# thenumbernine/lua-multigrid-poisson

Measured on AMD Instinct MI355X. Metric: V-cycles/sec + finest-smoother achieved HBM GB/s, 3D Poisson, higher is better.
Workload: dtype f32; 1 GPU; BASELINE configs[2]: 3D Poisson 512^3 per GPU, 7-point, RB-GS 2+2, V-cycle, trilinear P, 2x2x2-average R, consistent coarse boundary, per-cycle RMS-update err; parallelism=single GPU, levels=10

## Files before the change

lua-multigrid-poisson_amd/csrc/mgp_internal.h:

```cpp
#pragma once
#include <hip/hip_runtime.h>
#include <cstdint>

namespace mgp {

constexpr int kGhost3D = 1;
constexpr int kGhostZs = 5;
constexpr int kZsHaloPre = 5, kZsHaloPost = 4, kZsHaloCoarse = 3;

struct Geo {
    int nx, ny;
    int lx, ly;
    int hw, lhw;
    int64_t nz;
    int64_t H;
    int64_t P;
    int64_t z0;
    int64_t gnz;
};

constexpr int kRealF32D = 12;

hipError_t launch_init_point_charge(int rb, int dim, void* u, void* f, Geo g, int64_t cx, int64_t cy,
                                    int64_t cz, hipStream_t s);
// ... 11 lines not shown
                             const void* old, double* partials, Geo g, double h, double cl, bool gs, hipStream_t s);
bool fresh_supported(int rb, const Geo& g);
hipError_t launch_fresh_sweep(int rb, int dim, const void* f, void* u, Geo g, double h, double cl, hipStream_t s,
                              bool store_red = true);
bool post1_supported(int rb, const Geo& g, const Geo& gc);
hipError_t launch_post_first(int rb, int dim, int linear, void* u, const void* V, const void* f, Geo g, Geo gc,
                             double h, double cl, double clc, hipStream_t s);
hipError_t launch_residual_restrict(int rb, int dim, const void* u, const void* f, void* R, Geo g, Geo gc, double h,
                                    double cl, hipStream_t s);
bool bres_supported(int rb, const Geo& g);
hipError_t launch_black_residual_restrict(int rb, int dim, void* u, const void* f, void* R, Geo g, Geo gc, double h,
                                          double cl, hipStream_t s);
hipError_t launch_rb_sweep(int rb, int dim, const void* src, const void* f, void* dst, Geo g, double h, double cl,
                           bool store_red, hipStream_t s);
hipError_t launch_residual_field_v(int rb, int dim, const void* u, const void* f, void* r, Geo g, double h, double cl,
                                   hipStream_t s);
hipError_t launch_fw_restrict(int rb, int dim, const void* r, void* R, Geo g, Geo gc, double clc, hipStream_t s);
bool resfw_supported(int rb, int dim, const Geo& g, int gz, bool dist);
hipError_t launch_resfw(int rb, int dim, const void* u, const void* f, void* R, Geo g, Geo gc, double h, double cl,
                        double clc, int gz, hipStream_t s);
hipError_t launch_prolong_correct(int rb, int dim, int linear, void* u, const void* V, Geo g, Geo gc, double clc,
                                  hipStream_t s, bool black_only = false);
hipError_t launch_sqdiff_sum(int rb, const void* a, const void* b, int64_t n, double* partials, double* out,
                             hipStream_t s, int* ctr = nullptr);
hipError_t launch_nonfinite_check(int rb, const void* p, int64_t n, int id, int* first, hipStream_t s);
hipError_t launch_metrics(int rb, const void* psi, const void* old, int64_t n, double* partials, double* out,
                          hipStream_t s);
int resnorm_blocks(int rb, Geo g);
hipError_t launch_residual_norm(int rb, int dim, const void* u, const void* f, Geo g, double h, double cl,
                                double* partials, double* out, hipStream_t s);
int sum_scratch(int n);
hipError_t launch_sum_partials(const double* partials, int n, double* out, hipStream_t s, int* ctr = nullptr);

int defect_blocks(Geo g);
int refine_add_blocks(Geo g);
int refine_partials();
hipError_t launch_defect(int dim, const double* psi64, const double* f64, float* r32, float* u32_or_null, Geo g,
                         double h, double* partials, double* out, hipStream_t s);
hipError_t launch_refine_add(double* psi64, const float* e32, Geo g, double* partials, double* out, hipStream_t s);
hipError_t launch_refine_widen(const float* src, double* dst, int64_t n, hipStream_t s);
hipError_t launch_refine_narrow(const double* src, float* dst, int64_t n, hipStream_t s);

struct FusedTuning {
    bool wide = true;
    int ys_half = -1;
    int ys_rows = 32;
    int64_t wgs = 256;
    int patch_pre = 0, patch_post = -1;
    bool fwf = true;
    int post_zc = 256;
    bool split = true;
    bool split_cl = false;
    bool zpost_pre = true;
    bool stamp_r = false;
};
FusedTuning fused_tuning_from_env();

struct LaunchInfo {
    char name[96];
    int64_t grid;
};

struct FusedArgs {
    FusedTuning tu;
    LaunchInfo* info;
    bool pre;
    int linear;
    const void* src;
    const void* f;
    void* dst;
    const void* old;
    void* R;
    const void* V;
    double* partials;
    Geo g, gc;
    double h, cl, clc;
    int zc;
    int ghost;
};
bool fused_supported(int rb, int dim, int ns, const Geo& g, const FusedTuning& tu);
hipError_t prepare_kernels(int rb);
int fused_zc(int rb, const Geo& g, bool pre, bool clz, const FusedTuning& tu);
int fused_blocks(int rb, const Geo& g, int zc, bool clz, const FusedTuning& tu);
hipError_t launch_fused(int rb, const FusedArgs& a, hipStream_t s);
bool fused_fwf_supported(int rb, int dim, bool clz, bool dist, const FusedTuning& tu);

constexpr int kBlkMaxSweeps = 2;
constexpr int kBlkTile = 8;
constexpr int kBlkTile2D = 32;
struct BlockArgs {
    bool pre;
    int linear;
    int ns;
    const void* src;
    const void* f;
    void* dst;
    void* R;
    const void* V;
    Geo g, gc;
    double h, cl, clc;
};
bool block_supported(int rb, int dim, int ns, const Geo& g);
hipError_t launch_block(int rb, int dim, const BlockArgs& a, hipStream_t s);

struct Block2Args {
    bool pre;
// ... 62 lines not shown
```

lua-multigrid-poisson_amd/csrc/mgp_kernels.hip:

```cpp
#include "mgp_device.h"

#include <cstdio>
#include <cstdlib>
#include <type_traits>
#include <utility>

namespace mgp {
namespace {




constexpr unsigned kMaxBlocks = 1u << 20;
inline unsigned nblk_gs(int64_t n)
{
    const int64_t b = (n + kBlock - 1) / kBlock;
    return (unsigned)(b < (int64_t)kMaxBlocks ? (b > 0 ? b : 1) : kMaxBlocks);
}

template <typename T>
__global__ __launch_bounds__(kBlock) void k_init(T* __restrict__ u, T* __restrict__ f, Geo g, int64_t cx, int64_t cy,
                                                 int64_t cz, int dim3)
{
    const int64_t n = g.P * g.nz;
// ... 1232 lines not shown
#endif
#ifndef ZS_TYPRE_CL_F32
#define ZS_TYPRE_CL_F32 ZS_TYPRE_F32
#endif
#ifndef ZS_NPRE_CL_F32
#define ZS_NPRE_CL_F32 ZS_NPRE_F32
#endif
#ifndef ZS_TXPOST_W_F32
#define ZS_TXPOST_W_F32 128
#endif
#ifndef ZS_TYPOST_W_F32
#define ZS_TYPOST_W_F32 16
#endif
#ifndef ZS_NPOST_W_F32
#define ZS_NPOST_W_F32 ZS_NPOST_F32
#endif
template <typename T>
struct ZsTile;
template <>
struct ZsTile<float> {
    static constexpr int TXPRE = ZS_TXPRE_F32, TXPOST = ZS_TXPOST_F32, TYPRE = ZS_TYPRE_F32, TYPOST = ZS_TYPOST_F32,
                         NPRE = ZS_NPRE_F32, NPOST = ZS_NPOST_F32;
    static constexpr int TXPRE_CL = ZS_TXPRE_CL_F32, TYPRE_CL = ZS_TYPRE_CL_F32, NPRE_CL = ZS_NPRE_CL_F32;
    static constexpr int TXPOST_W = ZS_TXPOST_W_F32, TYPOST_W = ZS_TYPOST_W_F32, NPOST_W = ZS_NPOST_W_F32;
};
#ifndef ZS_TXPRE_F64
#define ZS_TXPRE_F64 32
#endif
#ifndef ZS_TXPOST_F64
#define ZS_TXPOST_F64 64
#endif
#ifndef ZS_TYPRE_F64
#define ZS_TYPRE_F64 32
#endif
#ifndef ZS_TYPOST_F64
#define ZS_TYPOST_F64 16
#endif
template <>
struct ZsTile<double> {
    static constexpr int TXPRE = ZS_TXPRE_F64, TXPOST = ZS_TXPOST_F64, TYPRE = ZS_TYPRE_F64, TYPOST = ZS_TYPOST_F64,
                         NPRE = 2, NPOST = 2;
    static constexpr int TXPRE_CL = TXPRE, TYPRE_CL = TYPRE, NPRE_CL = NPRE;
    static constexpr int TXPOST_W = TXPOST, TYPOST_W = TYPOST, NPOST_W = NPOST;
};
#ifndef ZS_NT
#define ZS_NT 0
#endif
constexpr bool kZsNTL = (ZS_NT & 1) != 0, kZsNTS = (ZS_NT & 2) != 0, kZsNTO = (ZS_NT & 5) != 0;
#ifndef ZS_PRE_RED_STORE
#define ZS_PRE_RED_STORE 0
#endif
constexpr bool kZsPreRed = ZS_PRE_RED_STORE != 0;

template <typename T, bool PRE, bool CLZ = true, bool WIDE = false, bool FWF = false>
struct ZsShape {
    static constexpr int N = PRE ? (CLZ ? ZsTile<T>::NPRE : ZsTile<T>::NPRE_CL)
                                 : (WIDE ? ZsTile<T>::NPOST_W : ZsTile<T>::NPOST);
    static constexpr int TX = PRE ? (CLZ ? ZsTile<T>::TXPRE : ZsTile<T>::TXPRE_CL)
                                  : (WIDE ? ZsTile<T>::TXPOST_W : ZsTile<T>::TXPOST);
    static constexpr int TY = PRE ? (CLZ ? ZsTile<T>::TYPRE : ZsTile<T>::TYPRE_CL)
                                  : (WIDE ? ZsTile<T>::TYPOST_W : ZsTile<T>::TYPOST);
    static constexpr int H = PRE ? (FWF ? 6 : 5) : 4;
#ifdef ZS_HX_FIXED
    static constexpr int HX = ZS_HX_FIXED;
#else
    static constexpr int HX = 2 * N * ((H + 2 * N - 1) / (2 * N));
#endif
    static constexpr int HWE = (TX + 2 * HX) / 2;
    static constexpr int G = HWE / N;
    static constexpr int HXG = HX / 2 / N;
    static constexpr int YE = TY + 2 * H;
    static constexpr int NT = G * YE;
    static constexpr int YEV = (YE + 1) / 2;
    static constexpr int NPAR = (G * YEV + 63) / 64 * 64;
    static constexpr bool PS = PRE ? ZS_PSPLIT_PRE != 0 : ZS_PSPLIT_POST != 0;
    static constexpr int NTL = PS ? 2 * NPAR : (NT + 63) / 64 * 64;
    static constexpr int YT0 = TY * G, YT1 = YT0 + 6 * G, YT2S = (YT1 + 63) / 64 * 64, YT2 = YT2S + 4 * G;
    static constexpr bool YROLE = ZS_YROLE && PRE && !PS && H == 5 && (YT2 + 63) / 64 * 64 <= NTL;
    static constexpr int GC = G - 2 * HXG, TC = TY * GC;
    static constexpr bool XROLE = YROLE && ZS_XROLE && TC % 64 == 0;
    static constexpr bool XPAIR = XROLE && ZS_XPAIR && GC == 8 && TY % 8 == 0 && HWE == 40;
    static __device__ __forceinline__ int xp_row(int q) { return (0x54450110 >> (4 * q)) & 15; }
    static __device__ __forceinline__ int xp_gx(int q) { return (0x64024620 >> (4 * q)) & 15; }
    static __device__ __forceinline__ int yrow(int t)
    {
        if (!YROLE) return t < NT ? t / G : -1;
        if (XPAIR && t < TC) return H + 8 * (t >> 6) + xp_row((t & 31) >> 2) + 2 * ((t >> 5) & 1);
        if (t < YT0) return H + (XROLE ? (t < TC ? t / GC : (t - TC) / (2 * HXG)) : t / G);
        if (t < YT1) {
            const int r = (t - YT0) / G;
            return r < 3 ? H - 3 + r : H + TY + r - 3;
        }
        if (t >= YT2S && t < YT2) {
            const int r = (t - YT2S) / G;
            return r < 2 ? H - 5 + r : H + TY + r + 1;
        }
        return -1;
    }
    static __device__ __forceinline__ int ycol(int t)
    {
        if (XROLE && t < YT0) {
            if (t < TC) return HXG + (XPAIR ? ((xp_gx((t & 31) >> 2) + (t & 3)) & 7) : t % GC);
            const int k = (t - TC) % (2 * HXG);
            return k < HXG ? k : GC + k;
        }
        return YROLE && t >= YT2S ? (t - YT2S) % G : t % G;
    }
    static constexpr int wave_role(int w)
    {
        return !YROLE || 64 * w < (XROLE ? TC : YT0) ? 0 : (64 * w < YT1 ? 1 : 2);
// ... 1169 lines not shown
#pragma unroll
            for (int e = 0; e < N; ++e) {
                rr[0][e] = pq == 0 ? rred[e] : rblk[e];
                rr[1][e] = pq == 0 ? rblk[e] : rred[e];
            }
            const int dq = q - (ST ? (Z0 & ~1) : Z0);
            if (dq >= 0 && dq <= zc && tile_xy)
                zs_restrict_avg<T, N>(rr, xr, acc, dq, zc, even_row, xs(q), R, (zz0 + q - 1) >> 1, gy >> 1, col.gm, cz0, gc);
            FB[sl(5)] = fb;
        }
    };

    if (wk == 0) {
        const int wrole = S::wave_role(lw);
        run(prefetch_a, [&](auto st, auto rt, const PF& cur, PF& nxt, int p) __attribute__((always_inline)) {
            step_a(st, rt, cur, nxt, p, decltype(st)::value ? wrole : 0);
        });
    } else if (wk == 1) {
        if (lw < SP::NTW)
            run(prefetch_b, [&](auto st, auto rt, const PF& cur, PF& nxt, int p) __attribute__((always_inline)) {
                step_b(st, rt, STY, p);
            });
        else
            run(prefetch_b, [&](auto st, auto rt, const PF& cur, PF& nxt, int p) __attribute__((always_inline)) {
                step_b(st, rt, GEN, p);
            });
    } else {
        run(
            [&](auto st, PF& r, int p) __attribute__((always_inline)) {
                if (!grp_b) prefetch_a(st, r, p);
            },
            [&](auto st, auto rt, const PF& cur, PF& nxt, int p) __attribute__((always_inline)) {
                if (!grp_b) step_a(st, rt, cur, nxt, p, 2);
                asm volatile("" ::: "memory");
                if (grp_b) step_b(st, rt, GEN, p);
            });
    }
}

template <typename T, bool ZSRC>
__global__ __launch_bounds__((ZsSplit<T>::NTL)) void k_zs_split(const T* __restrict__ src, const T* __restrict__ f,
                                                                 T* __restrict__ dst, T* __restrict__ R, Geo g, Geo gc,
                                                                 Op<T, 3> op, int zc, int gz, int patch)
{
    zs_split_body<T, ZSRC, true>(src, f, dst, R, g, gc, op, zc, gz, patch);
}

template <typename T>
__global__ __launch_bounds__((ZsSplit<T>::NTL)) void k_zs_split_cl(const T* __restrict__ f, T* __restrict__ dst,
                                                                    T* __restrict__ R, Geo g, Geo gc, Op<T, 3> op, int zc,
                                                                    int gz, int patch)
{
    zs_split_body<T, true, false>(nullptr, f, dst, R, g, gc, op, zc, gz, patch);
}

#ifndef YS_TX_F32
#define YS_TX_F32 1024
#endif
#ifndef YS_TX_F64
#define YS_TX_F64 512
#endif
template <typename T>
constexpr int ys_tx_full() { return sizeof(T) == 4 ? YS_TX_F32 : YS_TX_F64; }
template <typename T, bool PRE, int TXV = ys_tx_full<T>()>
struct YsShape {
    static constexpr int N = 16 / sizeof(T);
    static constexpr int TX = TXV;
    static constexpr int H = PRE ? 5 : 4;
    static constexpr int HX = 2 * N * ((H + 2 * N - 1) / (2 * N));
    static constexpr int HWE = TX / 2 + HX;
    static constexpr int G = HWE / N;
    static constexpr int HXG = HX / 2 / N;
    static constexpr int NTL = (G + 63) / 64 * 64;
    static constexpr int ES = 2 * G;
    static constexpr int OFF1 = 2 * ES, OFF2 = 4 * ES, OFF3 = 6 * ES, OFF4 = 10 * ES;
    static constexpr int CI = PRE ? 0 : TX / 2 + 16, CPAIRS = CI / 2, OFFC = 12 * ES;
    static constexpr size_t lds_floats = 12 * ES + 4 * CI;
    static_assert(CPAIRS <= 2 * NTL, "coarse staging: two pairs per thread");
    static_assert(NTL <= 1024, "too many threads");
    static_assert(2 * N * HXG >= H, "x halo too small");
};

#ifndef YS_PF
#define YS_PF 2
#endif
static_assert(YS_PF >= 1 && YS_PF <= 3, "prefetch distance 1..3");
template <typename T>
struct YsPrefetch {
    static constexpr int N = 16 / sizeof(T);
    Vec<T, N> u, f1, f2, o0, o1;
    Vec<T, 2> cv[2];
};

template <typename T, int N, bool CLZ, bool RES, bool AIN = false>
__device__ __forceinline__ void ys_cells(const Vec<T, N>& ym, const Vec<T, N>& cen, const Vec<T, N>& yp, T ep, T en,
                                         const Vec<T, N>& fv, const Vec<T, N>& uc, int o, int nby, int gm, int nx,
                                         bool xin, const Op<T, 2>& op, T (&out)[N], T (&ask)[N])
{
    if (!AIN) {
        ZsNb<T, N> nb;
        nb.yl = ym;
        nb.yr = yp;
        nb.ep = ep;
        nb.en = en;
        T t[N];
        zs_xsum<T, N>(cen, nb, o, t);
// ... 1673 lines not shown
template <int D>
static hipError_t pr_f32d(int linear, void* u, const void* V, Geo g, Geo gc, double clc, bool black, hipStream_t s)
{
    for (int color = black ? 1 : 0; color < 2; ++color) {
        const unsigned nb = nblk(g.H * g.nz);
        if (linear) k_prolong<float, D, 1, double><<<nb, kBlock, 0, s>>>((float*)u, (const float*)V, g, gc, clc, color);
        else k_prolong<float, D, 0, double><<<nb, kBlock, 0, s>>>((float*)u, (const float*)V, g, gc, clc, color);
        const hipError_t e = hipGetLastError();
        if (e != hipSuccess) return e;
    }
    return hipSuccess;
}

hipError_t launch_prolong_correct(int rb, int dim, int linear, void* u, const void* V, Geo g, Geo gc, double clc,
                                  hipStream_t s, bool black_only)
{
    if (rb == kRealF32D)
        return dim == 3 ? pr_f32d<3>(linear, u, V, g, gc, clc, black_only, s) : pr_f32d<2>(linear, u, V, g, gc, clc, black_only, s);
    if (rb == 8)
        return dim == 3 ? pr_t<double, 3>(linear, u, V, g, gc, clc, black_only, s)
                        : pr_t<double, 2>(linear, u, V, g, gc, clc, black_only, s);
    return dim == 3 ? pr_t<float, 3>(linear, u, V, g, gc, clc, black_only, s)
                    : pr_t<float, 2>(linear, u, V, g, gc, clc, black_only, s);
}


static int parse_patch(const char* v, int dflt)
{
    int px = 0, py = 0;
    if (!v) return dflt;
    if (std::sscanf(v, "%d,%d", &px, &py) != 2 || px < 1 || py < 1 || px > 255 || py > 255) return 0;
    return px | (py << 8);
}

FusedTuning fused_tuning_from_env()
{
    FusedTuning t;
    if (const char* v = std::getenv("MGP_ZS_WIDE")) t.wide = std::atoi(v) != 0;
    if (const char* v = std::getenv("MGP_YS_HALF")) t.ys_half = std::atoi(v);
    if (const char* v = std::getenv("MGP_YS_ROWS")) {
        const int r = std::atoi(v);
        t.ys_rows = r >= 8 && (r & 1) == 0 ? r : 32;
    }
    if (const char* v = std::getenv("MGP_ZS_WGS")) t.wgs = std::max<int64_t>(1, std::atoll(v));
    const char* vb = std::getenv("MGP_ZS_PATCH");
    const int both = parse_patch(vb, 0);
    t.patch_pre = parse_patch(std::getenv("MGP_ZS_PATCH_PRE"), both);
    t.patch_post = parse_patch(std::getenv("MGP_ZS_PATCH_POST"), vb ? both : -1);
    if (const char* v = std::getenv("MGP_ZS_FWF")) t.fwf = std::atoi(v) != 0;
    if (const char* v = std::getenv("MGP_ZS_POST_ZC")) t.post_zc = std::max(0, std::atoi(v));
    if (const char* v = std::getenv("MGP_ZS_SPLIT")) t.split = std::atoi(v) != 0;
    if (const char* v = std::getenv("MGP_ZS_SPLIT_CL")) t.split_cl = std::atoi(v) != 0;
    if (const char* v = std::getenv("MGP_ZPOST_PRE")) t.zpost_pre = std::atoi(v) != 0;
    if (const char* v = std::getenv("MGP_STAMP_R")) t.stamp_r = std::atoi(v) != 0;
    return t;
}

static int zs_patch(int patch, int tiles_x, int tiles_y, unsigned nb)
{
    if (patch == -1) patch = tiles_x * tiles_y >= 4096 ? 4 | (8 << 8) : 0;
    const int px = patch & 255, py = patch >> 8;
    if (!patch || tiles_x % px || tiles_y % py || nb <= 512) return 0;
    return patch;
}

static const char* tf(bool v) { return v ? "true" : "false"; }

template <typename T, bool PRE, int LINEAR, bool ERR, bool CLZ, bool WIDE = false>
static hipError_t zs_launch(const FusedArgs& a, hipStream_t s)
{
    using S = ZsShape<T, PRE, CLZ, WIDE, PRE && LINEAR == 2>;
    const Op<T, 3> op = make_op<T, 3>(a.h, a.cl);
    const unsigned nb = (unsigned)((a.g.nx / S::TX) * (a.g.ny / S::TY) * (a.g.nz / a.zc));
    if (a.info) {
        std::snprintf(a.info->name, sizeof a.info->name, "k_zs<%s, %s, %d, %s, %s, %s>", sizeof(T) == 4 ? "float" : "double",
                      tf(PRE), LINEAR, tf(ERR), tf(CLZ), tf(WIDE));
        a.info->grid = (int64_t)nb * S::NTL;
    }
    k_zs<T, PRE, LINEAR, ERR, CLZ, WIDE><<<nb, S::NTL, S::lds_bytes, s>>>((const T*)a.src, (const T*)a.f, (T*)a.dst,
                                                                           (const T*)(a.old ? a.old : a.dst), (T*)a.R,
                                                                           (const T*)a.V, a.partials, a.g, a.gc,
                                                                           op, (T)a.clc, a.zc, a.ghost,
                                                                           zs_patch(PRE ? a.tu.patch_pre : a.tu.patch_post,
                                                                                    a.g.nx / S::TX, a.g.ny / S::TY, nb));
    return hipGetLastError();
}

template <bool ZSRC>
static hipError_t zs_split_launch(const FusedArgs& a, hipStream_t s)
{
    using SP = ZsSplit<float>;
    using S = SP::S;
    const Op<float, 3> op = make_op<float, 3>(a.h, a.cl);
    const unsigned nb = (unsigned)((a.g.nx / S::TX) * (a.g.ny / S::TY) * (a.g.nz / a.zc));
    if (a.info) {
        std::snprintf(a.info->name, sizeof a.info->name, "k_zs_split<float, %s>", tf(ZSRC));
        a.info->grid = (int64_t)nb * SP::NTL;
    }
    k_zs_split<float, ZSRC><<<nb, SP::NTL, SP::lds_bytes, s>>>((const float*)a.src, (const float*)a.f, (float*)a.dst,
                                                                (float*)a.R, a.g, a.gc, op, a.zc, a.ghost,
                                                                zs_patch(a.tu.patch_pre, a.g.nx / S::TX, a.g.ny / S::TY, nb));
    return hipGetLastError();
}

static hipError_t zs_split_cl_launch(const FusedArgs& a, hipStream_t s)
{
    using SP = ZsSplit<float>;
    using S = SP::S;
    const Op<float, 3> op = make_op<float, 3>(a.h, a.cl);
    const unsigned nb = (unsigned)((a.g.nx / S::TX) * (a.g.ny / S::TY) * (a.g.nz / a.zc));
    if (a.info) {
        std::snprintf(a.info->name, sizeof a.info->name, "k_zs_split_cl<float>");
        a.info->grid = (int64_t)nb * SP::NTL;
    }
    k_zs_split_cl<float><<<nb, SP::NTL, SP::lds_bytes, s>>>((const float*)a.f, (float*)a.dst, (float*)a.R, a.g, a.gc, op, a.zc,
                                                           a.ghost,
                                                           zs_patch(a.tu.patch_pre, a.g.nx / S::TX, a.g.ny / S::TY, nb));
    return hipGetLastError();
}

#ifndef ZS_WIDE_CL
#define ZS_WIDE_CL 0
#endif
static bool zs_wide(int rb, const Geo& g, bool clz, const FusedTuning& tu)
{
    if (rb != 4 || (!clz && !ZS_WIDE_CL) || !tu.wide) return false;
    return g.nx % ZsTile<float>::TXPOST_W == 0 && g.ny % ZsTile<float>::TYPOST_W == 0;
}

static int ys_tx(int rb, const Geo& g, const FusedTuning& tu);

template <typename T, bool PRE, int LINEAR, bool ERR, bool CLZ, int TXV>
static hipError_t ys_launch_tx(const FusedArgs& a, hipStream_t s)
{
    using S = YsShape<T, PRE, TXV>;
    const Op<T, 2> op = make_op<T, 2>(a.h, a.cl);
    const unsigned nb = (unsigned)((a.g.nx / S::TX) * (a.g.ny / a.zc));
    if (a.info) {
        std::snprintf(a.info->name, sizeof a.info->name, "k_ys<%s, %s, %d, %s, %s, %d>", sizeof(T) == 4 ? "float" : "double",
                      tf(PRE), LINEAR, tf(ERR), tf(CLZ), TXV);
        a.info->grid = (int64_t)nb * S::NTL;
    }
    k_ys<T, PRE, LINEAR, ERR, CLZ, TXV><<<nb, S::NTL, 0, s>>>((const T*)a.src, (const T*)a.f, (T*)a.dst,
                                                         (const T*)(a.old ? a.old : a.dst), (T*)a.R, (const T*)a.V,
                                                         a.partials, a.g, a.gc, op, (T)a.clc, a.zc);
    return hipGetLastError();
}

template <typename T, bool PRE, int LINEAR, bool ERR, bool CLZ>
static hipError_t ys_launch(const FusedArgs& a, hipStream_t s)
{
    constexpr int F = ys_tx_full<T>();
    return ys_tx(sizeof(T), a.g, a.tu) == F ? ys_launch_tx<T, PRE, LINEAR, ERR, CLZ, F>(a, s)
                                      : ys_launch_tx<T, PRE, LINEAR, ERR, CLZ, F / 2>(a, s);
}

template <typename T, bool CLZ>
static hipError_t fused_dispatch_2d(const FusedArgs& a, hipStream_t s)
{
    const bool err = a.partials != nullptr;
    if (a.pre) return a.linear ? ys_launch<T, true, 1, false, CLZ>(a, s) : ys_launch<T, true, 0, false, CLZ>(a, s);
    if (a.linear) return err ? ys_launch<T, false, 1, true, CLZ>(a, s) : ys_launch<T, false, 1, false, CLZ>(a, s);
    return err ? ys_launch<T, false, 0, true, CLZ>(a, s) : ys_launch<T, false, 0, false, CLZ>(a, s);
}

template <typename T, bool CLZ>
static hipError_t fused_dispatch(const FusedArgs& a, hipStream_t s)
{
    const bool err = a.partials != nullptr;
#ifdef ZS_CL_AS_CLZ
    if (a.pre) return a.linear ? zs_launch<T, true, 1, false, true>(a, s) : zs_launch<T, true, 0, false, true>(a, s);
#endif
    if constexpr (std::is_same<T, float>::value && CLZ) {
        if (a.pre && a.linear == 2)
            return a.src ? zs_launch<T, true, 2, false, CLZ>(a, s) : zs_launch<T, true, 2, true, CLZ>(a, s);
    }
    if (a.pre && a.linear == 2) return hipErrorInvalidValue;
    if constexpr (std::is_same<T, float>::value && CLZ) {
        if (a.pre && !a.linear && a.tu.split) return a.src ? zs_split_launch<false>(a, s) : zs_split_launch<true>(a, s);
    }
    if constexpr (std::is_same<T, float>::value && !CLZ) {
        if (a.pre && !a.linear && !a.src && a.tu.split && a.tu.split_cl) return zs_split_cl_launch(a, s);
    }
    if (a.pre && !a.src)
        return a.linear ? zs_launch<T, true, 1, true, CLZ>(a, s) : zs_launch<T, true, 0, true, CLZ>(a, s);
    if (a.pre) return a.linear ? zs_launch<T, true, 1, false, CLZ>(a, s) : zs_launch<T, true, 0, false, CLZ>(a, s);
    if constexpr (std::is_same<T, float>::value && CLZ) {
        if (zs_wide(4, a.g, true, a.tu)) {
            if (a.linear)
                return err ? zs_launch<T, false, 1, true, CLZ, true>(a, s) : zs_launch<T, false, 1, false, CLZ, true>(a, s);
            return err ? zs_launch<T, false, 0, true, CLZ, true>(a, s) : zs_launch<T, false, 0, false, CLZ, true>(a, s);
        }
    }
    if constexpr (std::is_same<T, float>::value && !CLZ && ZS_WIDE_CL) {
        if (!err && zs_wide(4, a.g, false, a.tu))
            return a.linear ? zs_launch<T, false, 1, false, CLZ, true>(a, s) : zs_launch<T, false, 0, false, CLZ, true>(a, s);
    }
    if (a.linear) return err ? zs_launch<T, false, 1, true, CLZ>(a, s) : zs_launch<T, false, 1, false, CLZ>(a, s);
    return err ? zs_launch<T, false, 0, true, CLZ>(a, s) : zs_launch<T, false, 0, false, CLZ>(a, s);
}

static void zs_tile(int rb, int& tx, int& ty, int pre = -1, bool clz = true, bool wide = false)
{
    const int xa = rb == 4 ? ZsTile<float>::TXPRE : ZsTile<double>::TXPRE;
    const int xc = rb == 4 ? ZsTile<float>::TXPRE_CL : ZsTile<double>::TXPRE_CL;
    const int xb = rb == 4 ? ZsTile<float>::TXPOST : ZsTile<double>::TXPOST;
    const int a = rb == 4 ? ZsTile<float>::TYPRE : ZsTile<double>::TYPRE;
    const int ac = rb == 4 ? ZsTile<float>::TYPRE_CL : ZsTile<double>::TYPRE_CL;
    const int b = rb == 4 ? ZsTile<float>::TYPOST : ZsTile<double>::TYPOST;
    const int xp = clz ? xa : xc, yp = clz ? a : ac;
    auto mx = [](int u, int v, int w) { return u > v ? (u > w ? u : w) : (v > w ? v : w); };
    tx = pre < 0 ? mx(xa, xb, xc) : (pre ? xp : xb);
    ty = pre < 0 ? mx(a, b, ac) : (pre ? yp : b);
    if (pre == 0 && wide) {
        tx = ZsTile<float>::TXPOST_W;
        ty = ZsTile<float>::TYPOST_W;
    }
}

static int ys_rows(const Geo& g, const FusedTuning& tu)
{
    int r = tu.ys_rows;
    while (r > 8 && g.ny % r != 0) r /= 2;
    return r;
}

static int ys_tx(int rb, const Geo& g, const FusedTuning& tu)
{
    const int mode = tu.ys_half;
    const int64_t target = tu.wgs;
    const int full = rb == 4 ? ys_tx_full<float>() : ys_tx_full<double>();
    if (mode == 0 || g.nx % (full / 2) != 0) return full;
    if (mode == 1 || g.nx % full != 0) return full / 2;
    return (int64_t)(g.nx / full) * (g.ny / ys_rows(g, tu)) < target ? full / 2 : full;
}

bool fused_supported(int rb, int dim, int ns, const Geo& g, const FusedTuning& tu)
{
    if (dim == 2)
        return ns == 2 && g.nz == 1 && g.nx % ys_tx(rb, g, tu) == 0 && g.ny >= 16 && g.ny % ys_rows(g, tu) == 0;
    if (dim != 3 || ns != 2) return false;
// ... 10 lines not shown
    const int64_t target = tu.wgs;
    const int64_t tiles = (int64_t)(g.nx / TX) * (g.ny / TY);
    int64_t chunks = 1;
    while (tiles * chunks < target && g.nz / (chunks * 2) >= 16) chunks *= 2;
    while (!pre && tu.post_zc > 0 && g.nz / chunks > tu.post_zc && g.nz / (chunks * 2) >= 16) chunks *= 2;
    return (int)(g.nz / chunks);
}

int fused_blocks(int rb, const Geo& g, int zc, bool clz, const FusedTuning& tu)
{
    if (g.gnz == 1 && g.nz == 1) return (g.nx / ys_tx(rb, g, tu)) * (g.ny / zc);
    int TX, TY;
    zs_tile(rb, TX, TY, 0, clz, zs_wide(rb, g, clz, tu));
    return (int)((int64_t)(g.nx / TX) * (g.ny / TY) * (g.nz / zc));
}

int fused_halo(bool pre) { return pre ? 5 : 4; }

bool fused_fwf_supported(int rb, int dim, bool clz, bool dist, const FusedTuning& tu)
{
    return rb == 4 && dim == 3 && clz && !dist && tu.fwf;
}

template <typename T, bool CLZ>
static hipError_t fused_attr()
{
    const int pre = (int)ZsShape<T, true, CLZ>::lds_bytes, post = (int)ZsShape<T, false, CLZ>::lds_bytes;
    const auto A = hipFuncAttributeMaxDynamicSharedMemorySize;
    if constexpr (std::is_same<T, float>::value && CLZ) {
        const int w = (int)ZsShape<T, true, CLZ, false, true>::lds_bytes;
        hipError_t e = hipFuncSetAttribute((const void*)k_zs<T, true, 2, false, CLZ>, A, w);
        if (e == hipSuccess) e = hipFuncSetAttribute((const void*)k_zs<T, true, 2, true, CLZ>, A, w);
        if (e != hipSuccess) return e;
    }
    if constexpr (std::is_same<T, float>::value && CLZ) {
        const int w = (int)ZsShape<T, false, CLZ, true>::lds_bytes;
        hipError_t e = hipFuncSetAttribute((const void*)k_zs<T, false, 0, false, CLZ, true>, A, w);
        if (e == hipSuccess) e = hipFuncSetAttribute((const void*)k_zs<T, false, 0, true, CLZ, true>, A, w);
        if (e == hipSuccess) e = hipFuncSetAttribute((const void*)k_zs<T, false, 1, false, CLZ, true>, A, w);
        if (e == hipSuccess) e = hipFuncSetAttribute((const void*)k_zs<T, false, 1, true, CLZ, true>, A, w);
        if (e != hipSuccess) return e;
    }
    if constexpr (std::is_same<T, float>::value && !CLZ && ZS_WIDE_CL) {
        const int w = (int)ZsShape<T, false, CLZ, true>::lds_bytes;
        hipError_t e = hipFuncSetAttribute((const void*)k_zs<T, false, 0, false, CLZ, true>, A, w);
        if (e == hipSuccess) e = hipFuncSetAttribute((const void*)k_zs<T, false, 1, false, CLZ, true>, A, w);
        if (e != hipSuccess) return e;
    }
    hipError_t e = hipFuncSetAttribute((const void*)k_zs<T, true, 0, false, CLZ>, A, pre);
    if constexpr (std::is_same<T, float>::value && CLZ) {
        const int w = (int)ZsSplit<float>::lds_bytes;
        if (e == hipSuccess) e = hipFuncSetAttribute((const void*)k_zs_split<float, false>, A, w);
        if (e == hipSuccess) e = hipFuncSetAttribute((const void*)k_zs_split<float, true>, A, w);
    }
    if constexpr (std::is_same<T, float>::value && !CLZ) {
        if (e == hipSuccess)
            e = hipFuncSetAttribute((const void*)k_zs_split_cl<float>, A, (int)ZsSplit<float>::lds_bytes);
    }
    if (e == hipSuccess) e = hipFuncSetAttribute((const void*)k_zs<T, true, 1, false, CLZ>, A, pre);
    if (e == hipSuccess) e = hipFuncSetAttribute((const void*)k_zs<T, true, 0, true, CLZ>, A, pre);
    if (e == hipSuccess) e = hipFuncSetAttribute((const void*)k_zs<T, true, 1, true, CLZ>, A, pre);
    if (e == hipSuccess) e = hipFuncSetAttribute((const void*)k_zs<T, false, 0, false, CLZ>, A, post);
    if (e == hipSuccess) e = hipFuncSetAttribute((const void*)k_zs<T, false, 0, true, CLZ>, A, post);
    if (e == hipSuccess) e = hipFuncSetAttribute((const void*)k_zs<T, false, 1, false, CLZ>, A, post);
    if (e == hipSuccess) e = hipFuncSetAttribute((const void*)k_zs<T, false, 1, true, CLZ>, A, post);
    return e;
}

#ifdef TAIL_PROF
constexpr int kTailStaticLds = 1024;
#else
constexpr int kTailStaticLds = 0;
#endif
template <typename T>
static hipError_t tail_c_attr();

template <typename T, int D>
static hipError_t tail_attr()
{
    hipError_t e = hipFuncSetAttribute((const void*)k_tail<T, D, 0>, hipFuncAttributeMaxDynamicSharedMemorySize,
                                       (int)kTailMaxLds - kTailStaticLds);
    if (e == hipSuccess)
        e = hipFuncSetAttribute((const void*)k_tail<T, D, 1>, hipFuncAttributeMaxDynamicSharedMemorySize,
                                (int)kTailMaxLds - kTailStaticLds);
    return e;
}

template <typename T>
static hipError_t blk_attr();

hipError_t prepare_kernels(int rb)
{
    hipError_t e = hipSuccess;
#define MGP_CHAIN(x) \
    if (e == hipSuccess) e = (x)
    if (rb == 4) {
        MGP_CHAIN((fused_attr<float, true>()));
        MGP_CHAIN((fused_attr<float, false>()));
        MGP_CHAIN((tail_attr<float, 2>()));
        MGP_CHAIN((tail_attr<float, 3>()));
        MGP_CHAIN((tail_c_attr<float>()));
        MGP_CHAIN((blk_attr<float>()));
        MGP_CHAIN((blk2_attr(4)));
    } else {
        MGP_CHAIN((fused_attr<double, true>()));
        MGP_CHAIN((fused_attr<double, false>()));
// ... 415 lines not shown
```

Before: 1075 V-cycles/s (512^3-cell slabs, whole job).

## Add wave-specialized split POST kernel for fused prolong-correct plus two sweeps

Adds a new fused post-smoothing kernel that divides the workgroup's waves into two groups. Group A does the trilinear prolongation correction and the first two red-black half-sweeps. Group B stages coarse-grid values, runs the last two half-sweeps, stores the result and accumulates the error norm. The groups hand off through rotating LDS slots that include staged f rows, pipelined along z. The goal is better overlap and lower per-wave register pressure than the monolithic wide POST kernel on large grids (at least 2^27 cells by default). The cost is more LDS use and extra barriers, and correctness depends on subtle slot and parity bookkeeping.

```diff
diff --git a/lua-multigrid-poisson_amd/csrc/mgp_internal.h b/lua-multigrid-poisson_amd/csrc/mgp_internal.h
--- a/lua-multigrid-poisson_amd/csrc/mgp_internal.h
+++ b/lua-multigrid-poisson_amd/csrc/mgp_internal.h
@@ -87,6 +87,8 @@
     bool split = true;
     bool split_cl = false;
     bool zpost_pre = true;
+    bool split_post = true;
+    int64_t split_post_min_cells = (int64_t)1 << 27;
     bool stamp_r = false;
 };
 FusedTuning fused_tuning_from_env();
diff --git a/lua-multigrid-poisson_amd/csrc/mgp_kernels.hip b/lua-multigrid-poisson_amd/csrc/mgp_kernels.hip
--- a/lua-multigrid-poisson_amd/csrc/mgp_kernels.hip
+++ b/lua-multigrid-poisson_amd/csrc/mgp_kernels.hip
@@ -1308,10 +1308,11 @@
 #endif
 constexpr bool kZsPreRed = ZS_PRE_RED_STORE != 0;
 
-template <typename T, bool PRE, bool CLZ = true, bool WIDE = false, bool FWF = false>
+template <typename T, bool PRE, bool CLZ = true, bool WIDE = false, bool FWF = false, int NF = 0>
 struct ZsShape {
-    static constexpr int N = PRE ? (CLZ ? ZsTile<T>::NPRE : ZsTile<T>::NPRE_CL)
-                                 : (WIDE ? ZsTile<T>::NPOST_W : ZsTile<T>::NPOST);
+    static constexpr int N = NF ? NF
+                                : (PRE ? (CLZ ? ZsTile<T>::NPRE : ZsTile<T>::NPRE_CL)
+                                       : (WIDE ? ZsTile<T>::NPOST_W : ZsTile<T>::NPOST));
     static constexpr int TX = PRE ? (CLZ ? ZsTile<T>::TXPRE : ZsTile<T>::TXPRE_CL)
                                   : (WIDE ? ZsTile<T>::TXPOST_W : ZsTile<T>::TXPOST);
     static constexpr int TY = PRE ? (CLZ ? ZsTile<T>::TYPRE : ZsTile<T>::TYPRE_CL)
@@ -2587,6 +2588,398 @@
                                                                     int gz, int patch)
 {
     zs_split_body<T, true, false>(nullptr, f, dst, R, g, gc, op, zc, gz, patch);
+}
+
+template <typename T>
+struct ZsSplitPost {
+    using S = ZsShape<T, false, true, true, false, 4>;
+    static_assert(S::N == 4 && S::H == 4 && S::HXG == 1 && S::NS3 == 2 && !S::PS && !S::YROLE, "POST's wide tile, 16-byte columns");
+    static constexpr int G = S::G, NA = S::NT, NA2 = G * (S::TY + 4), NA3 = NA2 + 2 * G;
+    static constexpr int BROWS = S::TY + 2, GC = G - 2 * S::HXG, NBT = G * S::TY, NB = NBT + 2 * GC;
+    static constexpr int NWA = NA / 64, NWB = NB / 64, MA = NA - 64 * NWA;
+    static constexpr int NW = NWA + NWB + 1, NTL = 64 * NW, WLAST = NW - 1;
+    static constexpr unsigned BMASK = 0x25A;
+    static_assert(NWA == 6 && NWB == 5 && NB == 64 * NWB && MA > 0 && NW == 12, "wave order");
+    static __device__ __forceinline__ int wave_kind(int w) { return w == WLAST ? 2 : (int)((BMASK >> w) & 1u); }
+    static __device__ __forceinline__ int local_wave(int w)
+    {
+        const unsigned below = (1u << w) - 1u;
+        return __builtin_popcount(((BMASK >> w) & 1u) ? (BMASK & below) : (~BMASK & below));
+    }
+    static_assert(NA2 <= 64 * NWA, "A's last wave holds rows d >= 3 only");
+    static __device__ __forceinline__ int a_yrow(int t)
+    {
+        if (t < NA2) return 2 + t / G;
+        if (t < NA3) return t - NA2 < G ? 1 : S::YE - 2;
+        if (t < NA) return t - NA3 < G ? 0 : S::YE - 1;
+        return -1;
+    }
+    static __device__ __forceinline__ int b_yrow(int t)
+    {
+        if (t < NBT) return S::H + t / G;
+        return t - NBT < GC ? S::H - 1 : S::H + S::TY;
+    }
+    static __device__ __forceinline__ int b_ycol(int t) { return t < NBT ? t % G : S::HXG + (t - NBT) % GC; }
+    static constexpr int SLOT = S::SLOT, OFF1 = 2 * SLOT, OFF2 = 4 * SLOT, OFF3 = 8 * SLOT, OFFC = 10 * SLOT;
+    static constexpr int FSLOT = BROWS * S::HWE;
+    static constexpr int OFFFR = OFFC + 4 * S::CSLOT, OFFFB = OFFFR + 4 * FSLOT;
+    static constexpr size_t lds_bytes = (size_t)(OFFFB + 4 * FSLOT) * sizeof(T);
+    static constexpr int EG = (S::TX + 8) / 4, ENT = (EG * S::YE + 63) / 64 * 64;
+    static_assert(OFFC % 4 == 0 && S::CPAIRS <= 2 * NB, "coarse staging: two pairs per thread of B");
+    static_assert(NTL <= 1024 && NW <= 12, "too many waves for 168 VGPRs");
+    static_assert(lds_bytes + ENT * sizeof(double) <= 160 * 1024, "LDS");
+    static_assert(ENT <= 1024 && ENT - 512 <= NTL, "the sum's first level within the workgroup");
+};
+
+template <typename T, bool ERR>
+__global__ __launch_bounds__((ZsSplitPost<T>::NTL)) void k_zs_split_post(const T* __restrict__ src, const T* __restrict__ f,
+                                                                          T* __restrict__ dst, const T* old,
+                                                                          const T* __restrict__ V,
+                                                                          double* __restrict__ partials, Geo g, Geo gc,
+                                                                          Op<T, 3> op, T clc, int zc, int gz, int patch)
+{
+    using SP = ZsSplitPost<T>;
+    using S = typename SP::S;
+    constexpr int N = S::N, H = S::H, HWE = S::HWE, G = S::G, YE = S::YE, SLOT = S::SLOT, TX = S::TX, TY = S::TY;
+    using VT = Vec<T, N>;
+    using PF = ZsPrefetch<T, N>;
+    constexpr int PFD = 1, NPF = PFD + 1, UNR = 4;
+    extern __shared__ __align__(16) unsigned char zs_smem[];
+    T* const lds = reinterpret_cast<T*>(zs_smem);
+    const int tid = threadIdx.x;
+
+    const int tiles_x = g.nx / TX, tiles_y = g.ny / TY;
+    const int b = xcd_remap(blockIdx.x, gridDim.x);
+    const int tile = b % (tiles_x * tiles_y);
+    const int Z0 = (b / (tiles_x * tiles_y)) * zc;
+    int tx_, ty_;
+    zs_tile_xy(tile, tiles_x, patch, tx_, ty_);
+    const int X0 = tx_ * TX, Y0 = ty_ * TY;
+    const int hw = g.hw, Hh = (int)g.H;
+    const int z0 = (int)g.z0, gnz = (int)g.gnz, cz0 = (int)gc.z0;
+    const int64_t P = g.P;
+    const int qlo = -gz, qhi = (int)g.nz - 1 + gz;
+
+    const int wv = __builtin_amdgcn_readfirstlane(tid >> 6), lane = tid & 63;
+    const int wk = SP::wave_kind(wv), lw = SP::local_wave(wv);
+    const bool grp_b = wk == 1;
+    const int lt = wk == 2 ? 64 * SP::NWA + lane : 64 * lw + lane;
+    const int yr_ = grp_b ? SP::b_yrow(lt) : SP::a_yrow(lt);
+    const bool on = yr_ >= 0;
+    const int gx = on ? (grp_b ? SP::b_ycol(lt) : lt % G) : 0, ye = on ? yr_ : 0;
+    const int gy = Y0 - H + ye;
+    const int m0 = gx * N;
+    ZsCol col;
+    col.lrow = ye * HWE + m0;
+    col.lym = (ye > 0 ? ye - 1 : ye) * HWE + m0;
+    col.lyp = (ye < YE - 1 ? ye + 1 : ye) * HWE + m0;
+    col.gm = (X0 - S::HX) / 2 + m0;
+    col.x_first = gx == 0;
+    col.x_last = gx == G - 1;
+    col.lxm = col.x_first ? col.lrow : col.lrow - N;
+    col.lxp = col.x_last ? col.lrow : col.lrow + N;
+    const bool in_xy = on && gy >= 0 && gy < g.ny && col.gm >= 0 && col.gm < hw;
+    col.xin = true;
+    const int cgy = gy < 0 ? 0 : (gy >= g.ny ? g.ny - 1 : gy);
+    const int cgm = col.gm < 0 ? 0 : (col.gm > hw - N ? hw - N : col.gm);
+    const int goff = cgy * hw + cgm;
+    const bool tile_xy = on && ye >= H && ye < H + TY && gx >= S::HXG && gx < G - S::HXG;
+    const int ydist = ye < H ? H - ye : (ye >= H + TY ? ye - (H + TY) + 1 : 0);
+    const bool need_f1 = !ZS_FHALO || ydist <= H - 1, need_f2 = !ZS_FHALO || ydist <= H - 2;
+    const bool frow = on && ye >= H - 1 && ye <= H + TY;
+    const int lf = frow ? (ye - (H - 1)) * HWE + m0 : 0;
+    auto fslot = [&](int off, int q) { return lds + off + (q & 3) * SP::FSLOT + lf; };
+    const int zlo = Z0 - H;
+    const ZsDiag<T> dz = {};
+    const int p_end = Z0 + zc + 4;
+    auto inz = [&](int q) { return z0 + q >= 0 && z0 + q < gnz; };
+    auto pcl = [&](int q) { return q < qlo ? qlo : (q > qhi ? qhi : q); };
+    auto slot = [&](int off, int ns, int q) { return lds + off + (q & (ns - 1)) * SLOT; };
+    const int rowpar = (gy + z0) & 1;
+    auto par = [&](int q) { return rowpar ^ (q & 1); };
+    const VT vz = vzero<T, N>();
+
+    for (int i = tid; i < (int)(SP::lds_bytes / sizeof(T)); i += SP::NTL) lds[i] = (T)0;
+    __syncthreads();
+
+    const int Ia = X0 / 2 - 8, Ja = Y0 / 2 - 3;
+    auto ckl = [&](int K) { return K < 0 ? 0 : (K >= gc.gnz ? gc.gnz - 1 : K); };
+    auto cslot = [&](int K) { return lds + SP::OFFC + (K & 3) * S::CSLOT; };
+    int coff[2], cpar[2];
+#pragma unroll
+    for (int i = 0; i < 2; ++i) {
+        const int t = lt + i * SP::NB;
+        const int J = Ja + t / (S::CI / 2), I = Ia + 2 * (t % (S::CI / 2));
+        const bool ok = grp_b && t < S::CPAIRS && J >= 0 && J < gc.ny && I >= 0 && I < gc.nx;
+        coff[i] = ok ? J * gc.hw + (I >> 1) : -1;
+        cpar[i] = (I + J) & 1;
+    }
+    auto cload = [&](PF& r, int K) {
+        K = ckl(K);
+        const T* const pl = V + (int64_t)(K - cz0) * gc.P;
+#pragma unroll
+        for (int i = 0; i < 2; ++i) {
+            r.cv[i].v[0] = r.cv[i].v[1] = (T)0;
+            if (coff[i] >= 0) {
+                const int ce = (cpar[i] + K) & 1;
+                r.cv[i].v[0] = pl[coff[i] + ce * (int)gc.H];
+                r.cv[i].v[1] = pl[coff[i] + (ce ^ 1) * (int)gc.H];
+            }
+        }
+    };
+    auto cstore = [&](const PF& r, int K) {
+        T* const sl = cslot(ckl(K));
+#pragma unroll
+        for (int i = 0; i < 2; ++i) {
+            const int t = lt + i * SP::NB;
+            if (t < S::CPAIRS) vstore<T, 2>(sl + 2 * t, r.cv[i]);
+        }
+    };
+    auto crow = [&](int K, int J, T (&c)[N + 2]) {
+        const T* const sl = cslot(ckl(K)) + (J - Ja) * S::CI + (cgm - Ia);
+        const Vec<T, N> mid = vload<T, N>(sl);
+        c[0] = vload_lds_whole<T, N>(sl - N).v[N - 1];
+#pragma unroll
+        for (int e = 0; e < N; ++e) c[e + 1] = mid.v[e];
+        c[N + 1] = vload_lds_whole<T, N>(sl + N).v[0];
+    };
+    if (grp_b) {
+        PF r;
+        const int K = (z0 + zlo) >> 1;
+        for (int k = K - 1; k <= K + 1; ++k) {
+            cload(r, k);
+            cstore(r, k);
+        }
+    }
+    __syncthreads();
+
+    int ps = zlo, pe = p_end - 1;
+    ps = ps > 6 - z0 ? ps : 6 - z0;
+    ps = ps > qlo + 4 ? ps : qlo + 4;
+    pe = pe < gnz - 2 - z0 ? pe : gnz - 2 - z0;
+    pe = pe < qhi - PFD ? pe : qhi - PFD;
+    ps += (UNR - (ps - zlo) % UNR) % UNR;
+    pe -= (pe - ps + 1) % UNR;
+    if (pe < ps || ((z0 | Z0) & 1) || ((z0 + Z0) & 3)) ps = pe = zlo - 1;
+    const std::false_type GEN;
+    const std::true_type STY;
+    auto run = [&](auto&& prefetch, auto&& first_steady, auto&& step) __attribute__((always_inline)) {
+        PF pb[NPF];
+#pragma unroll
+        for (int k = 0; k < NPF; ++k) pb[k].f1 = pb[k].f2 = vz;
+#pragma unroll
+        for (int k = 0; k < PFD; ++k) prefetch(GEN, pb[k], zlo + k);
+        int p = zlo;
+        auto group = [&](auto st, int p0, int plim) __attribute__((always_inline)) {
+            zs_unroll<UNR>([&](auto kk) __attribute__((always_inline)) {
+                constexpr int k = decltype(kk)::value;
+                if (p0 + k <= plim) {
+                    step(st, std::integral_constant<int, (k & 3)>(), pb[k % NPF], pb[(k + PFD) % NPF], p0 + k);
+                    lds_barrier();
+                }
+            });
+        };
+        for (; p < ps; p += UNR) group(GEN, p, p + UNR);
+        if (p <= pe) first_steady(p);
+        for (; p <= pe; p += UNR) group(STY, p, p + UNR);
+        for (; p <= p_end; p += UNR) group(GEN, p, p_end);
+    };
+
+    const T* const src_black = src + Hh;
+    auto prefetch_a = [&](auto st, PF& r, int p) __attribute__((always_inline)) {
+        constexpr bool ST = decltype(st)::value;
+        if (ST) {
+            const int64_t pP = (int64_t)p * P;
+            r.u = gload<T, N, kZsNTL>(src_black + pP + goff);
+            if (need_f1) r.f1 = gload<T, N, kZsNTL>(f + (pP - P) + goff);
+            if (need_f2) r.f2 = gload<T, N, kZsNTL>(f + (pP - 2 * P) + Hh + goff);
+        } else {
+            r.u = gload<T, N, kZsNTL>(src_black + (int64_t)pcl(p) * P + goff);
+            if (need_f1) r.f1 = gload<T, N, kZsNTL>(f + (int64_t)pcl(p - 1) * P + goff);
+            if (need_f2) r.f2 = gload<T, N, kZsNTL>(f + (int64_t)pcl(p - 2) * P + Hh + goff);
+        }
+    };
+    VT W0[4], W1[4];
+    const bool corr_lane = (cgy >> 1) + ((cgy & 1) ? 1 : -1) >= 0 && (cgy >> 1) + ((cgy & 1) ? 1 : -1) < gc.ny && cgm > 0 &&
+                           cgm + N < gc.nx;
+    const bool corr_fast = __all(!on || corr_lane);
+    T BQ[2][2][N];
+    auto init_a = [&]() __attribute__((always_inline)) {
+#pragma unroll
+        for (int i = 0; i < 4; ++i) W0[i] = W1[i] = vz;
+#pragma unroll
+        for (int i = 0; i < 2 * 2 * N; ++i) (&BQ[0][0][0])[i] = (T)0;
+    };
+    const int bq_J = cgy >> 1;
+    int bq_Jn = (cgy & 1) ? bq_J + 1 : bq_J - 1;
+    const bool bq_oy = bq_Jn < 0 || bq_Jn >= gc.ny;
+    if (bq_oy) bq_Jn = bq_J;
+    auto bq_fill = [&](T (&bq)[2][N], int K) __attribute__((always_inline)) {
+        const int cp = cgy & 1;
+        T c0[N + 2], c1[N + 2];
+        crow(K, bq_J, c0);
+        crow(K, bq_Jn, c1);
+#pragma unroll
+        for (int q = 0; q < 2; ++q) zs_bq<T, N>(bq[q], c0, c1, q ^ cp, cgm, gc.nx, bq_oy, clc, corr_fast);
+    };
+    auto first_steady_a = [&](int p) __attribute__((always_inline)) {
+        const int K = (z0 + p) >> 1;
+        bq_fill(BQ[0], K);
+        bq_fill(BQ[1], K - 1);
+    };
+    auto step_a = [&](auto st, auto rt, auto full, const PF& cur, PF& nxt, int p) __attribute__((always_inline)) {
+        constexpr bool ST = decltype(st)::value, FULL = decltype(full)::value;
+        constexpr int RS = decltype(rt)::value;
+        auto sl = [](int k) constexpr { return (RS - k) & 3; };
+        if (!ST && p >= p_end) return;
+        if (ST) p = (p & ~1) | ((H + RS) & 1);
+        const int zz0 = ST ? (z0 & ~1) : z0;
+        zs_hold<T, N>(cur.u);
+        zs_hold<T, N>(cur.f1);
+        zs_hold<T, N>(cur.f2);
+        asm volatile("" ::: "memory");
+        if (ST || p + PFD <= p_end - 1) prefetch_a(st, nxt, p + PFD);
+        ZsNb<T, N> n1, n2;
+        VT a0 = cur.u;
+        if constexpr (ST) {
+            constexpr int KS = (RS >> 1) & 1, Q = 1 ^ (RS & 1);
+            if constexpr ((RS & 1) != 0) bq_fill(BQ[KS ^ 1], ((zz0 + p) >> 1) + 1);
+            const T w0 = (T)0.75, w1 = (T)0.25;
+#pragma unroll
+            for (int e = 0; e < N; ++e) a0.v[e] = a0.v[e] + (w0 * BQ[KS][Q][e] + w1 * BQ[KS ^ 1][Q][e]);
+        } else if (inz(p)) {
+            const int J = cgy >> 1, K = (zz0 + p) >> 1;
+            int Jn = (cgy & 1) ? J + 1 : J - 1;
+            int Kn = ((zz0 + p) & 1) ? K + 1 : K - 1;
+            const bool oy = Jn < 0 || Jn >= gc.ny, oz = Kn < 0 || Kn >= gc.gnz;
+            if (oy) Jn = J;
+            if (oz) Kn = K;
+            ZsCoarse<T, N> cc;
+            crow(K, J, cc.c00);
+            crow(K, Jn, cc.c10);
+            crow(Kn, J, cc.c01);
+            crow(Kn, Jn, cc.c11);
+            zs_correct<T, N, 1>(a0, cc, 1 ^ ((cgy + zz0 + p) & 1), cgm, gc.nx, oy, oz, clc,
+                                __all(!oy && !oz && cgm > 0 && cgm + N < gc.nx));
+        }
+        if (!ST && !inz(p)) a0 = vz;
+        W0[sl(0)] = a0;
+        zs_nb_load<T, N>(n1, slot(0, 2, p - 1), col);
+        VT o1 = zs_relax<T, N, true, ST>(W0[sl(2)], W0[sl(1)], W0[sl(0)], n1, cur.f1, col, par(p - 1), 0, g.nx, op, dz);
+        if (!ST && !inz(p - 1)) o1 = vz;
+        W1[sl(1)] = o1;
+        VT o2 = vz;
+        if constexpr (FULL) {
+            zs_nb_load<T, N>(n2, slot(SP::OFF1, 2, p - 2), col);
+            o2 = zs_relax<T, N, true, ST>(W1[sl(3)], W1[sl(2)], W1[sl(1)], n2, cur.f2, col, 1 ^ par(p - 2), 0, g.nx, op, dz);
+            if (!ST && !inz(p - 2)) o2 = vz;
+        }
+        if (in_xy) {
+            vstore<T, N>(slot(0, 2, p) + col.lrow, a0);
+            vstore<T, N>(slot(SP::OFF1, 2, p - 1) + col.lrow, o1);
+            if constexpr (FULL) vstore<T, N>(slot(SP::OFF2, 4, p - 2) + col.lrow, o2);
+            if (FULL && frow) {
+                vstore<T, N>(fslot(SP::OFFFR, p - 1), cur.f1);
+                vstore<T, N>(fslot(SP::OFFFB, p - 2), cur.f2);
+            }
+        }
+    };
+
+    auto prefetch_b = [&](auto st, PF& r, int p) __attribute__((always_inline)) {
+        constexpr bool ST = decltype(st)::value;
+        const int zz0 = ST ? (z0 & ~1) : z0;
+        if ((ST || p < p_end) && ((zz0 + p) & 1) == 0) cload(r, ((zz0 + p) >> 1) + 1);
+        if (ERR && tile_xy) {
+            const T* dp = old + (ST ? (int64_t)p * P - 5 * P : (int64_t)pcl(p - 5) * P);
+            r.o0 = gload<T, N, kZsNTO>(dp + goff);
+            r.o1 = gload<T, N, kZsNTO>(dp + Hh + goff);
+        }
+    };
+    VT W3[4];
+    double err[2], err1[2];
+    double esum[2] = {0.0, 0.0};
+    auto step_b = [&](auto st, auto rt, const PF& cur, PF& nxt, int p) __attribute__((always_inline)) {
+        constexpr bool ST = decltype(st)::value;
+        constexpr int RS = decltype(rt)::value;
+        auto sl = [](int k) constexpr { return (RS - k) & 3; };
+        if (ST) p = (p & ~1) | ((H + RS) & 1);
+        const int zz0 = ST ? (z0 & ~1) : z0;
+        if (ERR) {
+            zs_hold<T, N>(cur.o0);
+            zs_hold<T, N>(cur.o1);
+        }
+        zs_hold<T, 2>(cur.cv[0]);
+        zs_hold<T, 2>(cur.cv[1]);
+        asm volatile("" ::: "memory");
+        if ((ST || p < p_end) && ((zz0 + p) & 1) == 0) cstore(cur, ((zz0 + p) >> 1) + 1);
+        if (ST || p + PFD <= p_end) prefetch_b(st, nxt, p + PFD);
+        ZsNb<T, N> n3, n4;
+        const VT w2l = vload<T, N>(slot(SP::OFF2, 4, p - 5) + col.lrow), w2c = vload<T, N>(slot(SP::OFF2, 4, p - 4) + col.lrow),
+                 w2r = vload<T, N>(slot(SP::OFF2, 4, p - 3) + col.lrow);
+        const VT fr = vload<T, N>(fslot(SP::OFFFR, p - 4));
+        zs_nb_load<T, N>(n3, slot(SP::OFF2, 4, p - 4), col);
+        VT o3 = zs_relax<T, N, true, ST>(w2l, w2c, w2r, n3, fr, col, par(p - 4), 0, g.nx, op, dz);
+        if (!ST && !inz(p - 4)) o3 = vz;
+        if (in_xy) vstore<T, N>(slot(SP::OFF3, 2, p - 4) + col.lrow, o3);
+        W3[sl(4)] = o3;
+        const VT fb = vload<T, N>(fslot(SP::OFFFB, p - 5));
+        zs_nb_load<T, N>(n4, slot(SP::OFF3, 2, p - 5), col);
+        VT o4 = zs_relax<T, N, true, ST>(W3[sl(6)], W3[sl(5)], W3[sl(4)], n4, fb, col, 1 ^ par(p - 5), 0, g.nx, op, dz);
+        if (!ST && !inz(p - 5)) o4 = vz;
+        const int q = p - 5;
+        if (q >= Z0 && q < Z0 + zc && tile_xy) {
+            if (ERR) {
+#pragma unroll
+                for (int e = 0; e < N; ++e) {
+                    const double d0 = (double)W3[sl(5)].v[e] - (double)cur.o0.v[e];
+                    const double d1 = (double)o4.v[e] - (double)cur.o1.v[e];
+                    err[e >> 1] = __builtin_fma(d0, d0, err[e >> 1]);
+                    err1[e >> 1] = __builtin_fma(d1, d1, err1[e >> 1]);
+                }
+            }
+            T* dp = dst + (int64_t)q * P;
+            gstore<T, N, kZsNTS>(dp + goff, W3[sl(5)]);
+            gstore<T, N, kZsNTS>(dp + Hh + goff, o4);
+        }
+    };
+
+    if (wk == 0) {
+        init_a();
+        run(prefetch_a, first_steady_a, [&](auto st, auto rt, const PF& cur, PF& nxt, int p) __attribute__((always_inline)) {
+            step_a(st, rt, STY, cur, nxt, p);
+        });
+    } else if (wk == 1) {
+#pragma unroll
+        for (int i = 0; i < 4; ++i) W3[i] = vz;
+        err[0] = err[1] = err1[0] = err1[1] = 0.0;
+        run(prefetch_b, [](int) {}, step_b);
+        esum[0] = err[0] + err1[0];
+        esum[1] = err[1] + err1[1];
+    } else {
+        init_a();
+        run(prefetch_a, first_steady_a, [&](auto st, auto rt, const PF& cur, PF& nxt, int p) __attribute__((always_inline)) {
+            step_a(st, rt, GEN, cur, nxt, p);
+        });
+    }
+    if constexpr (ERR) {
+        __shared__ double red[SP::ENT];
+        for (int i = tid; i < SP::ENT; i += SP::NTL) red[i] = 0.0;
+        __syncthreads();
+        int t2 = tid;
+        asm volatile("" : "+v"(t2));
+        const int w2 = t2 >> 6, l2 = SP::local_wave(w2) * 64 + (t2 & 63);
+        const int y2 = SP::b_yrow(l2), x2 = SP::b_ycol(l2);
+        if (SP::wave_kind(w2) == 1 && y2 >= H && y2 < H + TY && x2 >= S::HXG && x2 < G - S::HXG) {
+            red[y2 * SP::EG + 2 * x2 - 1] = esum[0];
+            red[y2 * SP::EG + 2 * x2] = esum[1];
+        }
+        __syncthreads();
+        for (int w = 512; w > 0; w >>= 1) {
+            if (tid < w && tid + w < SP::ENT) red[tid] += red[tid + w];
+            __syncthreads();
+        }
+        if (tid == 0) partials[blockIdx.x] = red[0];
+    }
 }
 
 #ifndef YS_TX_F32
@@ -4366,6 +4759,8 @@
     if (const char* v = std::getenv("MGP_ZS_SPLIT")) t.split = std::atoi(v) != 0;
     if (const char* v = std::getenv("MGP_ZS_SPLIT_CL")) t.split_cl = std::atoi(v) != 0;
     if (const char* v = std::getenv("MGP_ZPOST_PRE")) t.zpost_pre = std::atoi(v) != 0;
+    if (const char* v = std::getenv("MGP_ZS_SPLIT_POST")) t.split_post = std::atoi(v) != 0;
+    if (const char* v = std::getenv("MGP_ZS_SPLIT_POST_MIN_CELLS")) t.split_post_min_cells = std::max<int64_t>(0, std::atoll(v));
     if (const char* v = std::getenv("MGP_STAMP_R")) t.stamp_r = std::atoi(v) != 0;
     return t;
 }
@@ -4433,6 +4828,24 @@
     return hipGetLastError();
 }
 
+template <bool ERR>
+static hipError_t zs_split_post_launch(const FusedArgs& a, hipStream_t s)
+{
+    using SP = ZsSplitPost<float>;
+    using S = SP::S;
+    const Op<float, 3> op = make_op<float, 3>(a.h, a.cl);
+    const unsigned nb = (unsigned)((a.g.nx / S::TX) * (a.g.ny / S::TY) * (a.g.nz / a.zc));
+    if (a.info) {
+        std::snprintf(a.info->name, sizeof a.info->name, "k_zs_split_post<float, %s>", tf(ERR));
+        a.info->grid = (int64_t)nb * SP::NTL;
+    }
+    k_zs_split_post<float, ERR><<<nb, SP::NTL, SP::lds_bytes, s>>>(
+        (const float*)a.src, (const float*)a.f, (float*)a.dst, (const float*)(a.old ? a.old : a.dst), (const float*)a.V,
+        a.partials, a.g, a.gc, op, (float)a.clc, a.zc, a.ghost,
+        zs_patch(a.tu.patch_post, a.g.nx / S::TX, a.g.ny / S::TY, nb));
+    return hipGetLastError();
+}
+
 #ifndef ZS_WIDE_CL
 #define ZS_WIDE_CL 0
 #endif
@@ -4501,6 +4914,10 @@
     if (a.pre) return a.linear ? zs_launch<T, true, 1, false, CLZ>(a, s) : zs_launch<T, true, 0, false, CLZ>(a, s);
     if constexpr (std::is_same<T, float>::value && CLZ) {
         if (zs_wide(4, a.g, true, a.tu)) {
+            static_assert(ZsSplitPost<float>::S::TX == ZsTile<float>::TXPOST_W && ZsSplitPost<float>::S::TY == ZsTile<float>::TYPOST_W,
+                          "the split POST runs on the wide tile");
+            if (a.linear && a.tu.split_post && (int64_t)a.g.nx * a.g.ny * a.g.nz >= a.tu.split_post_min_cells)
+                return err ? zs_split_post_launch<true>(a, s) : zs_split_post_launch<false>(a, s);
             if (a.linear)
                 return err ? zs_launch<T, false, 1, true, CLZ, true>(a, s) : zs_launch<T, false, 1, false, CLZ, true>(a, s);
             return err ? zs_launch<T, false, 0, true, CLZ, true>(a, s) : zs_launch<T, false, 0, false, CLZ, true>(a, s);
@@ -4617,6 +5034,9 @@
         const int w = (int)ZsSplit<float>::lds_bytes;
         if (e == hipSuccess) e = hipFuncSetAttribute((const void*)k_zs_split<float, false>, A, w);
         if (e == hipSuccess) e = hipFuncSetAttribute((const void*)k_zs_split<float, true>, A, w);
+        const int wp = (int)ZsSplitPost<float>::lds_bytes;
+        if (e == hipSuccess) e = hipFuncSetAttribute((const void*)k_zs_split_post<float, true>, A, wp);
+        if (e == hipSuccess) e = hipFuncSetAttribute((const void*)k_zs_split_post<float, false>, A, wp);
     }
     if constexpr (std::is_same<T, float>::value && !CLZ) {
         if (e == hipSuccess)
```

Result: faster. 1106 V-cycles/s (512^3-cell slabs, whole job) (median of 6 runs) (+2.9%).
